# TheShadow29/VidSitu

Hardware: AMD Instinct MI355X
Metric: clips/s (10s@32x224x224) SlowFast+TxEnc fwd+bwd (higher is better)
Workload: dtype bf16

## Files before the change

include/vidsitu_hip.h:

```cpp
#ifndef VIDSITU_HIP_H
#define VIDSITU_HIP_H

#include <stddef.h>
#include <stdint.h>

#ifdef __cplusplus
extern "C" {
#endif

typedef enum vs_status {
  VS_OK = 0,
  VS_ERR_BAD_ARG = -1,
  VS_ERR_UNSUPPORTED = -2,
  VS_ERR_WORKSPACE = -3,
  VS_ERR_LAUNCH = -4
} vs_status;

#define VS_CONV_AFFINE 1
#define VS_CONV_RESIDUAL 2
#define VS_CONV_RELU 4
#define VS_CONV_STATS 8
#define VS_CONV_NAIVE 16
#define VS_CONV_TILE(id) (((id) + 1) << 8)
#define VS_CONV_RING(ns) (((ns) & 7) << 16)
// ... 78 lines not shown
  const float* gamma;
  const float* beta;
  float* stats_partial;
  const void* bn_y2;
  int bn_y2_ld;
  const float* mean2;
  const float* invstd2;
  float* stats_partial2;
} vs_dgrad_epilogue;
int vs_conv_dgrad_ex(const void* dy, const void* wt, void* dx, const vs_conv_desc* d,
                     const vs_dgrad_epilogue* ep, void* workspace, size_t ws_bytes, void* stream);
int vs_weight_transpose(const void* w, void* wt, int Cout, int taps, int Cin, void* stream);
int vs_weight_transpose_batched(const void* src, void* dst, const int64_t* table, int n,
                                int64_t total, void* stream);
int vs_transpose_f32_batched(const float* src, float* dst, const int64_t* table, int n, int64_t total,
                             void* stream);
int vs_weight_transpose_tiled(const void* src, void* dst, const int64_t* table, const int64_t* tile_first,
                              int n, int64_t total_tiles, int elem_bytes, void* stream);

#define VS_WGRAD_NODEEP (1 << 12)
#define VS_WGRAD_FORCEDEEP (1 << 13)
size_t vs_conv_wgrad_workspace_bytes(const vs_conv_desc* d);
int vs_conv_wgrad(const void* dy, const void* x, float* dw, const vs_conv_desc* d,
                  void* workspace, size_t ws_bytes, void* stream);
typedef struct vs_wgrad_item {
  const void* dy;
  const void* x;
  float* dw;
  vs_conv_desc d;
} vs_wgrad_item;
int vs_conv_wgrad_group_ok(const vs_wgrad_item* items, int n);
size_t vs_conv_wgrad_group_workspace_bytes(const vs_wgrad_item* items, int n);
int vs_conv_wgrad_group(const vs_wgrad_item* items, int n, void* workspace, size_t ws_bytes, void* stream);
int vs_conv_wgrad_partial(const void* dy, const void* x, float* dw, const vs_conv_desc* d, void* slabs,
                          size_t slab_bytes, int* splits, void* stream);
int64_t vs_wgrad_reduce_blocks(int64_t elements);
int vs_wgrad_reduce(const float* slabs, float* dw, int64_t elements, int splits, void* stream);
int vs_wgrad_reduce_batched(const int64_t* table, int n_entries, int64_t total_blocks, void* stream);
int vs_wgrad_reduce_defer(int mode);
int vs_wgrad_reduce_flush(void);

int vs_bn_finalize(const float* partials, int nparts, double count, const float* gamma,
                   const float* beta, float* running_mean, float* running_var, float momentum,
                   float eps, float* scale, float* shift, float* mean, float* invstd, int C,
                   void* stream);
size_t vs_bn_finalize_workspace_bytes(void);
int vs_bn_finalize_ws(const float* partials, int nparts, double count, const float* gamma, const float* beta,
                      float* running_mean, float* running_var, float momentum, float eps, float* scale,
                      float* shift, float* mean, float* invstd, int C, void* workspace, size_t ws_bytes,
                      void* stream);
int vs_bn_partials_reduce(const float* partials, int nparts, float* out, int C, int G,
                          void* stream);
int vs_bn_apply(const void* y, const float* scale, const float* shift, const void* residual,
                void* out, int64_t rows, int C, int y_ld, int res_ld, int out_ld, int relu,
                void* stream);
int vs_bn_apply_mask(const void* y, const float* scale, const float* shift, const void* residual,
                     void* out, uint8_t* relu_bits, int64_t rows, int C, int y_ld, int res_ld,
                     int out_ld, void* stream);
int vs_bn_apply2(const void* y, const float* scale, const float* shift, const void* y2, const float* scale2,
                 const float* shift2, void* out, uint8_t* relu_bits, int64_t rows, int C, int y_ld, int y2_ld,
                 int out_ld, void* stream);
int vs_bn_bwd_reduce(const void* dz, const void* z, const void* y, const float* mean,
                     const float* invstd, const float* gamma, const float* beta, float* partial,
                     int64_t rows, int C, int dz_ld, int z_ld, int y_ld, int relu, void* stream);
int vs_bn_bwd_reduce_rows(int64_t rows, int C);
int vs_bn_bwd_finalize(const float* partial, int nparts, float* dgamma, float* dbeta, int C,
// ... 170 lines not shown
```

vidsitu_amd/_lib.py:

```python
import ctypes as C
import os
import subprocess

_HERE = os.path.dirname(os.path.abspath(__file__))
LIB_PATH = os.environ.get("VS_LIB_PATH") or os.path.join(_HERE, "libvidsitu_hip.so")
CSRC_DIR = os.path.join(_HERE, "csrc")

VS_CONV_AFFINE = 1
VS_CONV_RESIDUAL = 2
VS_CONV_RELU = 4
VS_CONV_STATS = 8
VS_CONV_NAIVE = 16


class ConvDesc(C.Structure):

    _fields_ = [
        (n, C.c_int32)
        for n in (
            "N Ti Hi Wi Cin To Ho Wo Cout kT kH kW sT sH sW pT pH pW x_ld y_ld res_ld flags"
        ).split()
    ]


# ... 17 lines not shown
SIGNATURES = {
    "vs_last_error_string": (C.c_char_p, []),
    "vs_version": (_i, []),
    "vs_launch_count": (_i64, []),
    "vs_pack_input": (_i, [_p, _i, _p, _i, _i, _i, _i, _i, _i, _p]),
    "vs_frames_u8_pack": (_i, [_p, _p, _p, _i, _i, _i, _i, _i, _i, _p, _p, _i, _p]),
    "vs_stem_conv_fwd": (_i, [_p, _p, _p, _i, _i, _i, _i, _i, _i, _i, _i, _p, _p, _p, _p]),
    "vs_stem_stats_rows": (_i, [_i, _i, _i, _i]),
    "vs_stem_wgrad_workspace_bytes": (_sz, [_i, _i, _i, _i, _i, _i]),
    "vs_stem_conv_wgrad": (_i, [_p, _p, _p, _i, _i, _i, _i, _i, _i, _i, _p, _sz, _p]),
    "vs_conv_fwd": (_i, [_p, _p, _p, _dp, _p, _p, _p, _p, _p, _sz, _p]),
    "vs_conv_stats_rows": (_i, [_dp]),
    "vs_conv_workspace_bytes": (_sz, [_dp, _i]),
    "vs_conv_plan": (_i, [_dp, _i, _p]),
    "vs_conv_aol_ok": (_i, [_dp]),
    "vs_conv_fwd_aol": (_i, [_p, _p, _p, _dp, _p, _p, _p, _p]),
    "vs_conv_wgrad_aol_ok": (_i, [_dp]),
    "vs_conv_wgrad_aol": (_i, [_p, _p, _p, _dp, _p, _p, _p, _sz, _p]),
    "vs_conv_fwd_bc_fusable": (_i, [_dp, _i]),
    "vs_conv_fwd_bc": (_i, [_p, _p, _dp, _p, _p, _p, _i, _p, _p, _p, _i, _p, _i, _i, _p]),
    "vs_conv_dgrad": (_i, [_p, _p, _p, _dp, _p, _p, _sz, _p]),
    "vs_conv_dgrad_bnstats_rows": (_i, [_dp]),
    "vs_conv_dgrad_bnstats": (_i, [_p, _p, _p, _dp, _p, _p, _i, _p, _p, _p, _p, _p, _p, _p, _sz, _p]),
    "vs_conv_dgrad_ex": (_i, [_p, _p, _p, _dp, C.POINTER(DgradEpilogue), _p, _sz, _p]),
    "vs_weight_transpose": (_i, [_p, _p, _i, _i, _i, _p]),
    "vs_weight_transpose_batched": (_i, [_p, _p, _p, _i, _i64, _p]),
    "vs_transpose_f32_batched": (_i, [_p, _p, _p, _i, _i64, _p]),
    "vs_weight_transpose_tiled": (_i, [_p, _p, _p, _p, _i, _i64, _i, _p]),
    "vs_conv_wgrad_workspace_bytes": (_sz, [_dp]),
    "vs_conv_wgrad": (_i, [_p, _p, _p, _dp, _p, _sz, _p]),
    "vs_conv_wgrad_group_ok": (_i, [C.POINTER(WgradItem), _i]),
    "vs_conv_wgrad_group_workspace_bytes": (_sz, [C.POINTER(WgradItem), _i]),
    "vs_conv_wgrad_group": (_i, [C.POINTER(WgradItem), _i, _p, _sz, _p]),
    "vs_conv_wgrad_partial": (_i, [_p, _p, _p, _dp, _p, _sz, C.POINTER(C.c_int), _p]),
    "vs_wgrad_reduce_blocks": (_i64, [_i64]),
    "vs_wgrad_reduce": (_i, [_p, _p, _i64, _i, _p]),
    "vs_wgrad_reduce_batched": (_i, [_p, _i, _i64, _p]),
    "vs_wgrad_reduce_defer": (_i, [_i]),
    "vs_wgrad_reduce_flush": (_i, []),
    "vs_bn_finalize": (_i, [_p, _i, _d, _p, _p, _p, _p, _f, _f, _p, _p, _p, _p, _i, _p]),
    "vs_bn_finalize_workspace_bytes": (_sz, []),
    "vs_bn_finalize_ws": (_i, [_p, _i, _d, _p, _p, _p, _p, _f, _f, _p, _p, _p, _p, _i, _p, _sz, _p]),
    "vs_bn_bwd_finalize_ws": (_i, [_p, _i, _p, _p, _i, _p, _sz, _p]),
    "vs_bn_partials_reduce": (_i, [_p, _i, _p, _i, _i, _p]),
    "vs_bn_apply": (_i, [_p, _p, _p, _p, _p, _i64, _i, _i, _i, _i, _i, _p]),
    "vs_bn_apply_mask": (_i, [_p, _p, _p, _p, _p, _p, _i64, _i, _i, _i, _i, _p]),
    "vs_bn_apply2": (_i, [_p, _p, _p, _p, _p, _p, _p, _p, _i64, _i, _i, _i, _i, _p]),
    "vs_bn_bwd_reduce": (_i, [_p, _p, _p, _p, _p, _p, _p, _p, _i64, _i, _i, _i, _i, _i, _p]),
    "vs_bn_bwd_reduce_rows": (_i, [_i64, _i]),
    "vs_bn_bwd_finalize": (_i, [_p, _i, _p, _p, _i, _p]),
    "vs_bn_bwd_apply": (
        _i,
        [_p, _p, _p, _p, _p, _p, _p, _p, _p, _p, _p, _i64, _i, _i, _i, _i, _i, _i, _i, _p],
    ),
    "vs_bn_bwd_apply2": (_i, [_p] * 16 + [_i64, _i, _i, _i, _i, _i, _i, _p]),
    "vs_residual_add_f32": (_i, [_p, _p, _p, _p, _p, _i64, _i, _i, _i, _i, _i, _i, _p]),
    "vs_maxpool_hw3s2_fwd": (_i, [_p, _p, _p, _i, _i, _i, _i, _i, _i, _i, _p]),
    "vs_maxpool_hw3s2_bwd": (_i, [_p, _p, _p, _i, _i, _i, _i, _i, _i, _i, _p]),
    "vs_bn_apply_maxpool": (_i, [_p, _p, _p, _p, _p, _i, _i, _i, _i, _i, _i, _i, _p]),
    "vs_bn_bwd_reduce_pool": (_i, [_p, _p, _p, _p, _p, _p, _p, _p, _i, _i, _i, _i, _i, _i, _i, _p]),
    "vs_bn_bwd_apply_pool": (_i, [_p, _p, _p, _p, _p, _p, _p, _p, _p, _p, _i, _i, _i, _i, _i, _i, _i, _i, _p]),
    "vs_maxpool_t_fwd": (_i, [_p, _p, _p, _i, _i, _i, _i, _i, _p]),
    "vs_maxpool_t_bwd": (_i, [_p, _p, _p, _i, _i, _i, _i, _i, _p]),
    "vs_avgpool_fwd": (_i, [_p, _p, _i, _i64, _i, _i, _i, _i, _p]),
    "vs_avgpool_bwd": (_i, [_p, _p, _i, _i64, _i, _i, _i, _i, _p]),
    "vs_linear_fwd": (_i, [_p, _p, _p, _p, _i, _i, _i, _i, _p]),
# ... 111 lines not shown
```

vidsitu_amd/csrc/conv_wgrad.hip:

```cpp
#include <stdlib.h>

#include "common.h"

#include <mutex>
#include <type_traits>
#include "glue_bodies.h"

typedef __attribute__((ext_vector_type(4))) short s16x4;
typedef __attribute__((address_space(3))) s16x4 lds_s16x4;

struct WgradP {
  const uint16_t* dy;
  const uint16_t* x;
  float* out;
  int P;
  int Cout, Kp, Cin, x_ld, dy_ld;
  int To, Ho, Wo, Ti, Hi, Wi;
  int kT, kH, kW, sT, sH, sW, pT, pH, pW;
  int tilesM, tilesN, S, rows_per_split;
  unsigned x_bytes, dy_bytes;
  int xcd_order;
  int dbg;
  const float* in_scale;
  const float* in_shift;
};

#define WG_OOB 0x80000000u

#define WG_ROWTAB 1024

__device__ __forceinline__ int wg_swz_chunk(int row) {
  return ((row & 3) << 1) | (((row >> 3) & 1) << 3);
}

template <int BM, int BN, int WM, int WN, int MODE>
__global__ __launch_bounds__(256) void conv_wgrad_kernel(WgradP p) {
  extern __shared__ __attribute__((aligned(16))) char smem[];
  constexpr int TM = BM / WM, TN = BN / WN;
  constexpr int MR = TM / 16, NR = TN / 16;
  constexpr int CM = BM / 8, CN = BN / 8;
  constexpr int RPM = 256 / CM, RPN = 256 / CN;
  constexpr int IM = (64 + RPM - 1) / RPM, IN = (64 + RPN - 1) / RPN;
  constexpr int IMG = 64 * 256;
  constexpr int STAGE = 2 * IMG;
  static_assert(WM * WN == 4, "4 waves");

  const int tid = threadIdx.x;
  int bid = blockIdx.x;
  if (p.xcd_order) {
    const int nwg = gridDim.x, q = nwg >> 3, r = nwg & 7, xcd = blockIdx.x & 7;
    bid = (xcd < r ? xcd * (q + 1) : r * (q + 1) + (xcd - r) * q) + (blockIdx.x >> 3);
  }
  const int ntile = p.tilesM * p.tilesN;
  const int s = bid / ntile;
  bid -= s * ntile;
  const int tn = bid % p.tilesN, tm = bid / p.tilesN;
  const int m0 = tm * BM, n0 = tn * BN;
  const int pbeg = s * p.rows_per_split;
  const int pend = min(p.P, pbeg + p.rows_per_split);

  int4* rowtab = (int4*)(smem + 2 * STAGE);

  const int ccm = tid % CM, rm = tid / CM;
  const int ccn = tid % CN, rn = tid / CN;
  const bool mcol_ok = (m0 + ccm * 8) < p.Cout;
  const int ncol = n0 + ccn * 8;
  const bool ncol_ok = ncol < p.Kp;
  int dt = 0, dh = 0, dw = 0, c0 = 0;
  if (MODE == 1 && ncol_ok) {
    const int tap = ncol / p.Cin;
    c0 = ncol - tap * p.Cin;
    dw = tap % p.kW;
    const int t2 = tap / p.kW;
    dh = t2 % p.kH;
    dt = t2 / p.kH;
  }

  u32x4 ra[IM], rb[IN];
  const __amdgpu_buffer_rsrc_t xsrc =
      __builtin_amdgcn_make_buffer_rsrc((void*)p.x, 0, (int)p.x_bytes, 0x00020000);
  const __amdgpu_buffer_rsrc_t dysrc =
      __builtin_amdgcn_make_buffer_rsrc((void*)p.dy, 0, (int)p.dy_bytes, 0x00020000);
  const unsigned dycol = (unsigned)((m0 + ccm * 8) * 2);
  const unsigned xtap = (MODE == 1)
// ... 117 lines not shown
      }
      __syncthreads();
    }
    const int nsteps = (cend - chunk0 + 63) >> 6;
    gload(chunk0, chunk0);
    __syncthreads();
    sstore(0);
    __syncthreads();
    for (int st = 0; st < nsteps - 1; ++st) {
      const int cur = st & 1;
      gload(chunk0 + (st + 1) * 64, chunk0);
      __builtin_amdgcn_sched_barrier(0);
      compute(cur);
      __builtin_amdgcn_sched_barrier(0);
      sstore(cur ^ 1);
      __syncthreads();
    }
    compute((nsteps - 1) & 1);
    __syncthreads();
  }

  float* dst = p.out + (long long)s * p.Cout * p.Kp;
#pragma unroll
  for (int a = 0; a < MR; ++a)
#pragma unroll
    for (int b = 0; b < NR; ++b) {
      const int col = n0 + wn * TN + b * 16 + li;
#pragma unroll
      for (int r = 0; r < 4; ++r) {
        const int row = m0 + wm * TM + a * 16 + g * 4 + r;
        if (row < p.Cout && col < p.Kp) dst[(long long)row * p.Kp + col] = acc[a][b][r];
      }
    }
}

template <int BM, int BN, int WM, int WN, int MODE, int NS, bool AOL = false, int ROWS = 64>
__device__ __forceinline__ void conv_wgrad_ring_body(const WgradP& p, const int blk, const int nblk) {
  static_assert(!AOL || MODE == 0, "apply on load: pointwise launches");
  static_assert(ROWS == 64, "stage depth (the half-depth variant of round 4 was measured slower and removed)");
  extern __shared__ __attribute__((aligned(16))) char smem[];
  constexpr int TM = BM / WM, TN = BN / WN;
  constexpr int MR = TM / 16, NR = TN / 16;
  constexpr int CM = BM / 8, CN = BN / 8;
  constexpr int IMG = ROWS * 256;
  constexpr int STAGE = 2 * IMG;
  constexpr int D = NS - 1;
  constexpr int RG = ROWS / 16;
  constexpr int L = 2 * RG;
  constexpr int SPC = WG_ROWTAB / ROWS;
  static_assert(WM * WN == 4, "4 waves");
  static_assert((D - 1) * L <= 63, "vmcnt range");

  const int tid = threadIdx.x;
  int bid = blk;
  if (p.xcd_order) {
    const int nwg = nblk, q = nwg >> 3, r = nwg & 7, xcd = blk & 7;
    bid = (xcd < r ? xcd * (q + 1) : r * (q + 1) + (xcd - r) * q) + (blk >> 3);
  }
  const int ntile = p.tilesM * p.tilesN;
  const int s = bid / ntile;
  bid -= s * ntile;
  const int tn = bid % p.tilesN, tm = bid / p.tilesN;
  const int m0 = tm * BM, n0 = tn * BN;
  const int pbeg = s * p.rows_per_split;
  const int pend = min(p.P, pbeg + p.rows_per_split);
  const int nsteps = (pend - pbeg + ROWS - 1) / ROWS;
// ... 1051 lines not shown
      int mx = 0;
      for (int x = 0; x < 8; ++x) {
        long long sl = 0;
        for (long long c = x; c < chunks; c += 8) sl = (c >> 3) * 32 + ((c == chunks - 1 && (pos & 31)) ? (pos & 31) : 32);
        g.jobend[x] = (unsigned short)sl;
        if ((int)sl > mx) mx = (int)sl;
      }
#ifdef VS_WGG_DEBUG
      for (int x = 0; x < 8; ++x) {
        fprintf(stderr, "xcd %d (%d slots):", x, (int)g.jobend[x]);
        for (int i = 0; i < cnt[x]; ++i) fprintf(stderr, " [slot %u p %u s %u t %u]", g.jobtab[x][i] >> 23, (g.jobtab[x][i] >> 18) & 31, (g.jobtab[x][i] >> 12) & 63, g.jobtab[x][i] & 4095);
        fprintf(stderr, "\n");
      }
      for (int a = 0; a < n; ++a) fprintf(stderr, "problem %d: tiles %d x %d S %d rps %d count %d\n", a, g.p[a].tilesM, g.p[a].tilesN, g.p[a].S, g.p[a].rows_per_split, g.count[a]);
#endif
      g.jobs = 1;
      grid = 8 * mx;
    }
  }
  static std::once_flag gattr;
  std::call_once(gattr, [] {
    (void)hipFuncSetAttribute((const void*)conv_wgrad_deep_group_kernel, hipFuncAttributeMaxDynamicSharedMemorySize, 160 * 1024);
  });
  const size_t smem = (size_t)WGD_NU * WGD_UNIT + 2 * WGD_TAB * sizeof(int2);
  hipLaunchKernelGGL(conv_wgrad_deep_group_kernel, dim3(grid), dim3(512), smem, (hipStream_t)stream, g);
  VS_CHECK_LAUNCH();
  if (r.n > 0) {
    hipLaunchKernelGGL(wgrad_reduce_group_kernel, dim3((unsigned)r.first[r.n]), dim3(256), 0, (hipStream_t)stream, r);
    VS_CHECK_LAUNCH();
  }
  return VS_OK;
}

static int wgrad_impl(const void* dy, const void* x, float* dw, const vs_conv_desc* d, void* workspace,
                      size_t ws_bytes, void* stream, bool reduce_now, int* splits_out,
                      const float* in_scale = nullptr, const float* in_shift = nullptr) {
  VS_CHECK_ARG(d && dy && x && dw, "null argument");
  VS_CHECK_ARG(d->Cin % 8 == 0 && d->Cout % 8 == 0, "Cin and Cout must be multiples of 8");
  VS_CHECK_ARG(d->x_ld % 8 == 0 && d->y_ld % 8 == 0, "row pitches must be multiples of 8");
  VS_CHECK_ARG((long long)d->N * d->Ti * d->Hi * d->Wi < (1ll << 31), "too many positions");
  const WgCfg c = wg_pick(d);
  const size_t need = vs_conv_wgrad_workspace_bytes(d);
  if (need > 0 && (workspace == nullptr || ws_bytes < need)) {
    vs_set_error("vs_conv_wgrad: workspace too small (%zu < %zu)", ws_bytes, need);
    return VS_ERR_WORKSPACE;
  }
  if (g_pending.have && ((const void*)g_pending.r.slabs == workspace || g_pending.r.dw == dw)) pending_flush();
  if (in_scale && !wgrad_aol_plan_ok(d)) {
    vs_set_error("vs_conv_wgrad_aol: apply on load is not built for this weight gradient (ask vs_conv_wgrad_aol_ok)");
    return VS_ERR_UNSUPPORTED;
  }
  WgradP p;
  {
    const int rc = wg_fill_params(p, dy, x, c.S > 1 ? (float*)workspace : dw, d, c);
    if (rc) return rc;
  }
  p.in_scale = in_scale;
  p.in_shift = in_shift;
  {
    static const int xo = [] { const char* e = getenv("VS_WGRAD_XCD"); return e ? atoi(e) : 1; }();
    p.xcd_order = xo && (c.tilesM * c.tilesN <= 32 || xo == 2 || (c.S % 8 == 0 && c.tilesM * c.tilesN <= 64));
    static const int dbg = [] { const char* e = getenv("VS_WGRAD_DBG"); return e ? atoi(e) : 0; }();
    p.dbg = dbg;
  }
  p.rows_per_split = c.rows_per_split;
  const bool dense = (d->kT * d->kH * d->kW == 1) && d->sT == 1 && d->sH == 1 && d->sW == 1 &&
                     d->pT == 0 && d->pH == 0 && d->pW == 0;
  const int mode = dense ? 0 : 1;
  hipStream_t st = (hipStream_t)stream;
  const int fring = (d->flags >> 16) & 7;
  int ring = fring == 1 ? 0 : (fring >= 2 ? (fring > 3 ? 3 : fring) : (c.bm == 128 ? 2 : 0));
  if (d->kT * d->kH * d->kW > 31) ring = 0;
  int rc;
  if (c.deep) {
    static std::once_flag dattr;
    std::call_once(dattr, [] {
      (void)hipFuncSetAttribute((const void*)conv_wgrad_deep_kernel<0, false>, hipFuncAttributeMaxDynamicSharedMemorySize, 160 * 1024);
      (void)hipFuncSetAttribute((const void*)conv_wgrad_deep_kernel<1, false>, hipFuncAttributeMaxDynamicSharedMemorySize, 160 * 1024);
      (void)hipFuncSetAttribute((const void*)conv_wgrad_deep_kernel<0, true>, hipFuncAttributeMaxDynamicSharedMemorySize, 160 * 1024);
      (void)hipFuncSetAttribute((const void*)conv_wgrad_deep_kernel<1, true>, hipFuncAttributeMaxDynamicSharedMemorySize, 160 * 1024);
    });
    static const int stag = [] { const char* e = getenv("VS_WGRAD_DEEP_STAG"); return e ? atoi(e) : 1; }();
    if (in_scale) {
      vs_set_error("vs_conv_wgrad_aol: not built for the deep-pipeline plan");
      return VS_ERR_UNSUPPORTED;
    }
    const size_t smem = (size_t)WGD_NU * WGD_UNIT + 2 * WGD_TAB * sizeof(int2);
    const int grid = p.tilesM * p.tilesN * p.S;
    if (stag && mode == 0) hipLaunchKernelGGL((conv_wgrad_deep_kernel<0, true>), dim3(grid), dim3(512), smem, st, p);
    else if (stag) hipLaunchKernelGGL((conv_wgrad_deep_kernel<1, true>), dim3(grid), dim3(512), smem, st, p);
    else if (mode == 0) hipLaunchKernelGGL((conv_wgrad_deep_kernel<0, false>), dim3(grid), dim3(512), smem, st, p);
    else hipLaunchKernelGGL((conv_wgrad_deep_kernel<1, false>), dim3(grid), dim3(512), smem, st, p);
    VS_CHECK_LAUNCH();
    rc = VS_OK;
// ... 43 lines not shown
```

vidsitu_amd/ops.py:

```python
import ctypes as C

import torch

from . import _lib
from ._lib import (
    VS_CONV_AFFINE,
    VS_CONV_NAIVE,
    VS_CONV_RELU,
    VS_CONV_RESIDUAL,
    VS_CONV_STATS,
    ConvDesc,
)

BF16 = torch.bfloat16


def _stream():
    return C.c_void_p(torch.cuda.current_stream().cuda_stream)


def _ptr(t):
    if t is None:
        return None
    if not t.is_cuda:
# ... 479 lines not shown
    return lambda: _lib.call("vs_wgrad_reduce", _ptr(ws), _ptr(out), n, S, _stream())


WGRAD_GROUP_MAX = 20


def _wgrad_items(items):
    arr = (_lib.WgradItem * len(items))()
    for i, (dy, x, k, s, p, out) in enumerate(items):
        if not out.permute(0, 2, 3, 4, 1).is_contiguous() or out.dtype != torch.float32:
            raise _lib.VsError("conv_wgrad out must be fp32 with [Cout][taps][Cin] memory")
        arr[i].dy, arr[i].x, arr[i].dw = dy.data_ptr(), x.data_ptr(), out.data_ptr()
        arr[i].d = make_desc(x.shape, act_ld(x), dy.shape, act_ld(dy), k, s, p, 0)
        _ptr(dy), _ptr(x), _ptr(out)
    return arr


def conv_wgrad_group_ok(items):
    if not 1 <= len(items) <= WGRAD_GROUP_MAX:
        return False
    return bool(_lib.load().vs_conv_wgrad_group_ok(_wgrad_items(items), len(items)))


def conv_wgrad_group(items):
    if _WHATIF_WGRAD:
        return
    arr = _wgrad_items(items)
    need = int(_lib.load().vs_conv_wgrad_group_workspace_bytes(arr, len(items)))
    ws = _workspace(need, items[0][0].device, "wgrad") if need else None
    _lib.call("vs_conv_wgrad_group", arr, len(items), _ptr(ws), C.c_size_t(ws.numel() if ws is not None else 0),
              _stream())


def conv_wgrad(dy, x, k, s, p, out=None, ring=0, batch=None, tile=None, slots=0, deep=True):
    cout, cin = dy.shape[1], x.shape[1]
    if out is None:
        out = torch.empty((cout, *k, cin), dtype=torch.float32, device=x.device).permute(0, 4, 1, 2, 3)
    elif not out.permute(0, 2, 3, 4, 1).is_contiguous() or out.dtype != torch.float32:
        raise _lib.VsError("conv_wgrad out must be fp32 with [Cout][taps][Cin] memory")
    if batch is not None:
        return batch.wgrad(dy, x, k, s, p, out, ring)
    if _WHATIF_WGRAD:
        return out
    flags = ((ring & 7) << 16) | (((tile + 1) << 8) if tile is not None else 0) | (((slots // 8) & 0xff) << 24)
    if not deep:
        flags |= 1 << 12
    elif deep == "force":
        flags |= 1 << 13
    d = make_desc(x.shape, act_ld(x), dy.shape, act_ld(dy), k, s, p, flags)
    need = _lib.load().vs_conv_wgrad_workspace_bytes(C.byref(d))
    ws = _workspace(need, x.device, "wgrad") if need else None
    _lib.call("vs_conv_wgrad", _ptr(dy), _ptr(x), _ptr(out), C.byref(d), _ptr(ws),
              C.c_size_t(ws.numel() if ws is not None else 0), _stream())
    return out


import os as _os
_WHATIF = int(_os.environ.get("VS_WHATIF", "0"))
_BN_TWO_LEVEL = int(_os.environ.get("VS_BN_TWO_LEVEL", "512"))
BN_FIN2 = _os.environ.get("VS_BN_FIN2", "1") != "0"
_fin_ws = [0]
_whatif_const = {}


def _fin_ws_bytes():
    if not _fin_ws[0]:
# ... 781 lines not shown
```

vidsitu_amd/trunk.py:

```python
import contextlib
import os

import torch
from torch import nn

from . import ops

STAGE_DEPTH = {50: (3, 4, 6, 3), 101: (3, 4, 23, 3), "tiny": (1, 0, 0, 1), "mini": (1, 1, 1, 1)}
TEMPORAL_KERNEL_BASIS = {
    "c2d": [[[1]], [[1]], [[1]], [[1]], [[1]]],
    "i3d": [[[5]], [[3]], [[3, 1]], [[3, 1]], [[1, 3]]],
    "slow": [[[1]], [[1]], [[1]], [[3]], [[3]]],
    "slowfast": [[[1], [5]], [[1], [3]], [[1], [3]], [[3], [3]], [[3], [3]]],
}
POOL1 = {
    "c2d": [[2, 1, 1]],
    "i3d": [[2, 1, 1]],
    "slow": [[1, 1, 1]],
    "slowfast": [[1, 1, 1], [1, 1, 1]],
}


class Conv3dP(nn.Module):

# ... 471 lines not shown
            else:
                sc = _Unit.fwd(self.branch1, self.branch1_bn, x, False, train=train, saved=saved)
        a = _Unit.fwd(b2.a, b2.a_bn, x, True, train=train, saved=saved)
        if sc_aff is not None:
            b = _Unit.fwd(b2.b, b2.b_bn, a, True, train=True, saved=saved)
            z = _Unit.fwd(b2.c, b2.c_bn, b, True, out=out, train=True, saved=saved, residual_affine=sc_aff)
            if saved is not None and len(saved) >= 4:
                saved[-1]["sc_rec"] = saved[-4]
            return z
        if train and self._aol_ok(a, saved):
            yb, aff = _Unit.fwd(b2.b, b2.b_bn, a, True, train=True, saved=saved, no_apply=True)
            z = _Unit.fwd(b2.c, b2.c_bn, yb, True, residual=sc, out=out, train=True, saved=saved, x_affine=aff)
            if self.has_sc and saved is not None and len(saved) >= 4:
                saved[-1]["sc_rec"] = saved[-4]
            return z
        if not train and self._bc_fusable(a):
            (sb, hb), (s_c, h_c) = b2.b_bn.fold, b2.c_bn.fold
            return ops.conv_fwd_bc(a, b2.b.w_bf16, b2.b.k, b2.b.s, b2.b.p, sb, hb, b2.c.w_bf16, s_c, h_c,
                                   residual=sc, relu=True, out=out)
        b = _Unit.fwd(b2.b, b2.b_bn, a, True, train=train, saved=saved)
        if ResBlock.residual_fp32 and not train:
            branch = _Unit.fwd(b2.c, b2.c_bn, b, False, train=False)
            res = sc if self.has_sc else getattr(x, "_vs_f32", x)
            z, z32 = ops.residual_add_f32(branch, res, relu=True, out16=out)
            z._vs_f32 = z32
            return z
        z = _Unit.fwd(b2.c, b2.c_bn, b, True, residual=sc, out=out, train=train, saved=saved)
        if self.has_sc and train and saved is not None and len(saved) >= 4:
            saved[-1]["sc_rec"] = saved[-4]
        return z

    def bwd(self, saved, dout, chain=False, carry=None):
        rc, rb, ra = saved.pop(), saved.pop(), saved.pop()
        sink = [] if self._wgrad_grouped(rc, rb, ra, saved[-1] if (self.has_sc and saved) else None, dout) else None
        res = self._bwd_units(saved, dout, chain, rc, rb, ra, sink)
        if sink:
            items = [(dy, x, c.k, c.s, c.p, c.weight.grad) for dy, x, c in sink]
            if carry is None:
                ops.conv_wgrad_group(items)
            else:
                carry["items"] += items
                carry["blocks"] += 1
                if carry["blocks"] >= ResBlock.group_span or len(carry["items"]) + 4 > ops.WGRAD_GROUP_MAX:
                    ResBlock.flush_wgrads(carry)
        return res

    @staticmethod
    def flush_wgrads(carry):
        if carry and carry["items"]:
            items = carry["items"]
            ops.conv_wgrad_group(items)
        if carry:
            carry["items"], carry["blocks"] = [], 0


    group_span = int(os.environ.get("VS_WGRAD_GROUP_SPAN", "3"))

    group_wgrads = os.environ.get("VS_WGRAD_GROUP", "1") != "0"
    group_max_positions = int(os.environ.get("VS_WGRAD_GROUP_MAXP", "1000000000"))
    group_min_channels = int(os.environ.get("VS_WGRAD_GROUP_MINC", "128"))

    def _wgrad_grouped(self, rc, rb, ra, rsc, dout):
        if (not ResBlock.group_wgrads or not dout.is_cuda or _Unit.wgrad_batch is not None or _Unit.split_wgrad_reduce
                or ResBlock.aol):
            return False
        recs = [r for r in (rc, rb, ra, rsc) if r is not None]
        key = ("wgg",) + tuple(tuple(r["y"].shape) for r in recs)
        hit = self.__dict__.setdefault("_bc_ok", {}).get(key)
        if hit is None:
            hit = True
            items = []
            for r in recs:
                c, y, x = r["conv"], r["y"], r["x"]
                if (c.is_stem or c.cin_pad != c.cin or c.bias is not None or r.get("x_affine") is not None
                        or c.cout < ResBlock.group_min_channels or not isinstance(x, torch.Tensor)
                        or not getattr(c.weight, "_vs_direct_grad", True)):
                    hit = False
                    break
                items.append((y, x, c.k, c.s, c.p, torch.empty(0)))
            if hit:
                hit = min(ops.act_rows(r["y"]) for r in recs) <= ResBlock.group_max_positions
            if hit:
                probe = [(y, x, k, s_, p, torch.empty((y.shape[1], *k, x.shape[1]), dtype=torch.float32,
                                                      device=y.device).permute(0, 4, 1, 2, 3)) for y, x, k, s_, p, _ in items]
                hit = ops.conv_wgrad_group_ok(probe)
            self._bc_ok[key] = hit
        return hit

    def _bwd_units(self, saved, dout, chain, rc, rb, ra, sink):
        cbits = rc.get("zbits")
        dy_sc = None
        if (self.has_sc and cbits is not None and ResBlock.fuse_sc_bwd and dout.is_cuda and saved
                and rc["conv"].bias is None and saved[-1]["conv"].bias is None and ops.bn_apply2_ok(rc["y"].shape[1])):
            rsc = saved[-1]
            units = []
            for r in (rc, rsc):
                bn = r["bn"]
                if bn.weight.grad is None:
                    bn.weight.grad = torch.zeros_like(bn.weight)
                if bn.bias.grad is None:
                    bn.bias.grad = torch.zeros_like(bn.bias)
                ops.bn_bwd_sums(dout, r["y"], r["mean"], r["invstd"], cbits, bn.weight.grad, bn.bias.grad,
                                partial=r.pop("bwd_partial", None))
                units.append((r["y"], r["mean"], r["invstd"], bn.weight, bn.weight.grad, bn.bias.grad))
            dy_c, dy_sc = ops.bn_bwd_apply2(dout, cbits, units[0], units[1])
            db, g = _Unit.bwd(rc, dout, producer=rb, dy_ready=dy_c, wgrad_sink=sink)
        else:
            db, g = _Unit.bwd(rc, dout, want_dres=cbits is None, producer=rb, wgrad_sink=sink)
        da, _ = _Unit.bwd(rb, db, producer=ra, wgrad_sink=sink)
        if self.has_sc:
            rsc = saved.pop()
            if ResBlock.accumulate_shortcut:
                dxa, _ = _Unit.bwd(ra, da, wgrad_sink=sink)
                if cbits is not None:
                    dx, _ = _Unit.bwd(rsc, dout, dz_bits=cbits, dx_residual=dxa, inplace=True, dy_ready=dy_sc, wgrad_sink=sink)
                else:
                    dx, _ = _Unit.bwd(rsc, g, masked=True, dx_residual=dxa, inplace=True, wgrad_sink=sink)
            else:
# ... 605 lines not shown
            par = self._fork_ctx(d[0].device)
            d_in = list(d)
            par.fork()
            for p in reversed(range(self.num_pathways)):
                with par.on(p):
                    if p == 1 and late is not None:
                        d[1] = late()
                    getattr(self.s1, f"pathway{p}_stem").bwd(saved, d[p])
            par.join(keep=d_in)
            assert not saved, "trunk backward did not consume every saved record"

    def _backward_stage(self, st, k):
        saved, d = st["saved"], st["d"]
        P = self.num_pathways
        stage = getattr(self, f"s{k}")
        fuse = getattr(self, f"s{k}_fuse", None) if self.multi else None
        if k == 2:
            for p in reversed(range(P)):
                if self.pool1[p][0] > 1:
                    rec = saved.pop()
                    d[p] = ops.maxpool_t_bwd(d[p], rec["tpool_idx"], rec["tpool_in"], rec["kt"])
        late = None
        if fuse is not None:
            d, late = self._fuse_bwd(saved, d, defer=VideoTrunk.fuse_on_fast)
        par = self._fork_ctx(d[0].device)
        d_in = list(d)
        par.fork()
        for p in reversed(range(P)):
            with par.on(p):
                if p == 1 and late is not None:
                    d[1] = late()
                g = d[p]
                blks = stage.blocks(p)
                carry = {"items": [], "blocks": 0}
                for i in reversed(range(len(blks))):
                    if isinstance(blks[i], ResBlock):
                        g = blks[i].bwd(saved, g, chain=i > 0, carry=carry)
                    else:
                        ResBlock.flush_wgrads(carry)
                        g = blks[i].bwd(saved, g)
                ResBlock.flush_wgrads(carry)
                d[p] = g
        par.join(keep=d_in)
        st["d"] = d

    fuse_on_fast = os.environ.get("VS_FUSE_ON_FAST", "1") != "0"

    def _fuse_bwd(self, saved, d, defer=False):
        d_cat, d_fast = d
        rec = saved.pop()
        cf = rec["conv"].cout
        cs = d_cat.shape[1] - cf
        run = lambda: _Unit.bwd(rec, ops.channel_slice(d_cat, cs, cf), dx_residual=d_fast)[0]
        if defer:
            return [ops.channel_slice(d_cat, 0, cs), None], run
        return [ops.channel_slice(d_cat, 0, cs), run()], None
```

Before: 730.2.

## Group narrow-channel wgrad convs into one multi-body kernel launch

Adds a grouped weight-gradient kernel that dispatches each block to one of several templated tile bodies, so ResBlocks whose channel count is below the wide-group threshold can batch their wgrad convolutions. Items are sorted by work size and launched together, followed by a single grouped split-K reduce, or one reduce per item. The Python side classifies blocks as wide or narrow, carries narrow items across blocks and flushes whenever the kind changes. The goal is fewer kernel launches and better GPU fill for the small fast-pathway convs, at the cost of a kernel with many bodies and possibly higher register and LDS use.

```diff
diff --git a/include/vidsitu_hip.h b/include/vidsitu_hip.h
--- a/include/vidsitu_hip.h
+++ b/include/vidsitu_hip.h
@@ -134,6 +134,11 @@
 int vs_conv_wgrad_group_ok(const vs_wgrad_item* items, int n);
 size_t vs_conv_wgrad_group_workspace_bytes(const vs_wgrad_item* items, int n);
 int vs_conv_wgrad_group(const vs_wgrad_item* items, int n, void* workspace, size_t ws_bytes, void* stream);
+#define VS_WGS_REDUCE_EACH 1
+int vs_conv_wgrad_group_small_ok(const vs_wgrad_item* items, int n);
+size_t vs_conv_wgrad_group_small_workspace_bytes(const vs_wgrad_item* items, int n);
+int vs_conv_wgrad_group_small(const vs_wgrad_item* items, int n, void* workspace, size_t ws_bytes, int flags,
+                              void* stream);
 int vs_conv_wgrad_partial(const void* dy, const void* x, float* dw, const vs_conv_desc* d, void* slabs,
                           size_t slab_bytes, int* splits, void* stream);
 int64_t vs_wgrad_reduce_blocks(int64_t elements);
diff --git a/vidsitu_amd/_lib.py b/vidsitu_amd/_lib.py
--- a/vidsitu_amd/_lib.py
+++ b/vidsitu_amd/_lib.py
@@ -73,6 +73,9 @@
     "vs_conv_wgrad_group_ok": (_i, [C.POINTER(WgradItem), _i]),
     "vs_conv_wgrad_group_workspace_bytes": (_sz, [C.POINTER(WgradItem), _i]),
     "vs_conv_wgrad_group": (_i, [C.POINTER(WgradItem), _i, _p, _sz, _p]),
+    "vs_conv_wgrad_group_small_ok": (_i, [C.POINTER(WgradItem), _i]),
+    "vs_conv_wgrad_group_small_workspace_bytes": (_sz, [C.POINTER(WgradItem), _i]),
+    "vs_conv_wgrad_group_small": (_i, [C.POINTER(WgradItem), _i, _p, _sz, _i, _p]),
     "vs_conv_wgrad_partial": (_i, [_p, _p, _p, _dp, _p, _sz, C.POINTER(C.c_int), _p]),
     "vs_wgrad_reduce_blocks": (_i64, [_i64]),
     "vs_wgrad_reduce": (_i, [_p, _p, _i64, _i, _p]),
diff --git a/vidsitu_amd/csrc/conv_wgrad.hip b/vidsitu_amd/csrc/conv_wgrad.hip
--- a/vidsitu_amd/csrc/conv_wgrad.hip
+++ b/vidsitu_amd/csrc/conv_wgrad.hip
@@ -34,7 +34,7 @@
 }
 
 template <int BM, int BN, int WM, int WN, int MODE>
-__global__ __launch_bounds__(256) void conv_wgrad_kernel(WgradP p) {
+__device__ __forceinline__ void conv_wgrad_body(const WgradP& p, const int blk, const int nblk) {
   extern __shared__ __attribute__((aligned(16))) char smem[];
   constexpr int TM = BM / WM, TN = BN / WN;
   constexpr int MR = TM / 16, NR = TN / 16;
@@ -46,10 +46,10 @@
   static_assert(WM * WN == 4, "4 waves");
 
   const int tid = threadIdx.x;
-  int bid = blockIdx.x;
+  int bid = blk;
   if (p.xcd_order) {
-    const int nwg = gridDim.x, q = nwg >> 3, r = nwg & 7, xcd = blockIdx.x & 7;
-    bid = (xcd < r ? xcd * (q + 1) : r * (q + 1) + (xcd - r) * q) + (blockIdx.x >> 3);
+    const int nwg = nblk, q = nwg >> 3, r = nwg & 7, xcd = blk & 7;
+    bid = (xcd < r ? xcd * (q + 1) : r * (q + 1) + (xcd - r) * q) + (blk >> 3);
   }
   const int ntile = p.tilesM * p.tilesN;
   const int s = bid / ntile;
@@ -233,6 +233,11 @@
         if (row < p.Cout && col < p.Kp) dst[(long long)row * p.Kp + col] = acc[a][b][r];
       }
     }
+}
+
+template <int BM, int BN, int WM, int WN, int MODE>
+__global__ __launch_bounds__(256) void conv_wgrad_kernel(WgradP p) {
+  conv_wgrad_body<BM, BN, WM, WN, MODE>(p, blockIdx.x, gridDim.x);
 }
 
 template <int BM, int BN, int WM, int WN, int MODE, int NS, bool AOL = false, int ROWS = 64>
@@ -1350,6 +1355,177 @@
   return VS_OK;
 }
 
+static int wg_xcd_order(const WgCfg& c) {
+  static const int xo = [] { const char* e = getenv("VS_WGRAD_XCD"); return e ? atoi(e) : 1; }();
+  return xo && (c.tilesM * c.tilesN <= 32 || xo == 2 || (c.S % 8 == 0 && c.tilesM * c.tilesN <= 64));
+}
+
+#define WGS_MAX 20
+struct WgSmallGroupP {
+  int n;
+  int first[WGS_MAX + 1];
+  int count[WGS_MAX];
+  int body[WGS_MAX];
+  WgradP p[WGS_MAX];
+};
+static_assert(sizeof(WgSmallGroupP) <= 4096, "kernel arguments");
+static_assert(WGS_MAX <= WGG_MAX, "one wgrad_reduce_group_kernel launch holds the slabs of a whole group");
+
+__global__ __launch_bounds__(256) void conv_wgrad_small_group_kernel(WgSmallGroupP g) {
+  const int b = blockIdx.x;
+  int j = 0;
+#pragma unroll
+  for (int i = 1; i < WGS_MAX; ++i)
+    if (i < g.n && b >= g.first[i]) j = i;
+  j = __builtin_amdgcn_readfirstlane(j);
+  const int blk = b - g.first[j], cnt = g.count[j];
+  if (blk >= cnt) return;
+  switch (__builtin_amdgcn_readfirstlane(g.body[j])) {
+    case 0: conv_wgrad_body<16, 64, 1, 4, 1>(g.p[j], blk, cnt); break;
+    case 1: conv_wgrad_body<16, 128, 1, 4, 1>(g.p[j], blk, cnt); break;
+    case 2: conv_wgrad_body<32, 64, 1, 4, 0>(g.p[j], blk, cnt); break;
+    case 3: conv_wgrad_body<32, 64, 1, 4, 1>(g.p[j], blk, cnt); break;
+    case 4: conv_wgrad_body<64, 64, 2, 2, 0>(g.p[j], blk, cnt); break;
+    case 5: conv_wgrad_body<64, 64, 2, 2, 1>(g.p[j], blk, cnt); break;
+    case 6: conv_wgrad_body<64, 128, 2, 2, 0>(g.p[j], blk, cnt); break;
+    case 7: conv_wgrad_body<64, 128, 2, 2, 1>(g.p[j], blk, cnt); break;
+    case 8: conv_wgrad_ring_body<128, 64, 2, 2, 0, 2>(g.p[j], blk, cnt); break;
+    case 9: conv_wgrad_ring_body<128, 64, 2, 2, 1, 2>(g.p[j], blk, cnt); break;
+    case 10: conv_wgrad_ring_body<128, 128, 2, 2, 1, 2>(g.p[j], blk, cnt); break;
+    default: break;
+  }
+}
+
+static int wgs_body(const WgCfg& c, int mode) {
+  static const int tab[][4] = {{16, 64, 1, 0},  {16, 128, 1, 1}, {32, 64, 0, 2},  {32, 64, 1, 3},
+                               {64, 64, 0, 4},  {64, 64, 1, 5},  {64, 128, 0, 6}, {64, 128, 1, 7},
+                               {128, 64, 0, 8}, {128, 64, 1, 9}, {128, 128, 1, 10}};
+  if (c.deep) return -1;
+  for (const auto& t : tab)
+    if (t[0] == c.bm && t[1] == c.bn && t[2] == mode) return t[3];
+  return -1;
+}
+
+static bool wg_dense(const vs_conv_desc* d) {
+  return (d->kT * d->kH * d->kW == 1) && d->sT == 1 && d->sH == 1 && d->sW == 1 && d->pT == 0 && d->pH == 0 &&
+         d->pW == 0;
+}
+
+static bool wgs_plan(const vs_wgrad_item* it, int n, WgCfg* cfg, int* body, size_t* slab_off, size_t* slab_total,
+                     int* order, size_t* smem) {
+  if (it == nullptr || n < 1 || n > WGS_MAX) return false;
+  size_t off = 0, lds = 0;
+  long long key[WGS_MAX], blocks = 0;
+  for (int j = 0; j < n; ++j) {
+    const vs_conv_desc* d = &it[j].d;
+    if (d->flags != 0 || d->Cin % 8 != 0 || d->Cout % 8 != 0 || d->x_ld % 8 != 0 || d->y_ld % 8 != 0) return false;
+    if ((long long)d->N * d->Ti * d->Hi * d->Wi >= (1ll << 31)) return false;
+    const int taps = d->kT * d->kH * d->kW;
+    const long long P = (long long)d->N * d->To * d->Ho * d->Wo;
+    const long long xb = (long long)d->N * d->Ti * d->Hi * d->Wi * d->x_ld * 2, db = P * d->y_ld * 2;
+    if (taps > 31 || P < 1 || xb >= (1ll << 31) || db >= (1ll << 31)) return false;
+    cfg[j] = wg_pick(d);
+    const int mode = wg_dense(d) ? 0 : 1;
+    body[j] = wgs_body(cfg[j], mode);
+    if (body[j] < 0) return false;
+    slab_off[j] = off;
+    if (cfg[j].S > 1) off += (size_t)cfg[j].S * d->Cout * taps * d->Cin * sizeof(float);
+    const size_t need = 2 * 2 * 64 * 256 + (mode ? 2 * WG_ROWTAB * sizeof(int2) : 0);
+    if (need > lds) lds = need;
+    const long long nb = (long long)cfg[j].tilesM * cfg[j].tilesN * cfg[j].S;
+    blocks += (nb + 7) / 8 * 8;
+    key[j] = (long long)cfg[j].rows_per_split * (cfg[j].bm + cfg[j].bn);
+    order[j] = j;
+  }
+  for (int a = 0; a < n; ++a)
+    for (int b = a + 1; b < n; ++b)
+      if (key[order[b]] > key[order[a]]) { const int t = order[a]; order[a] = order[b]; order[b] = t; }
+  *slab_total = off;
+  *smem = lds;
+  return blocks < (1ll << 31);
+}
+
+extern "C" int vs_conv_wgrad_group_small_ok(const vs_wgrad_item* items, int n) {
+  WgCfg cfg[WGS_MAX];
+  int body[WGS_MAX], order[WGS_MAX];
+  size_t off[WGS_MAX], tot, smem;
+  return wgs_plan(items, n, cfg, body, off, &tot, order, &smem) ? 1 : 0;
+}
+
+extern "C" size_t vs_conv_wgrad_group_small_workspace_bytes(const vs_wgrad_item* items, int n) {
+  WgCfg cfg[WGS_MAX];
+  int body[WGS_MAX], order[WGS_MAX];
+  size_t off[WGS_MAX], tot = 0, smem;
+  if (!wgs_plan(items, n, cfg, body, off, &tot, order, &smem)) return 0;
+  return tot;
+}
+
+extern "C" int vs_conv_wgrad_group_small(const vs_wgrad_item* items, int n, void* workspace, size_t ws_bytes, int flags,
+                                         void* stream) {
+  VS_CHECK_ARG(items != nullptr && n >= 1 && n <= WGS_MAX, "1 .. 20 items");
+  VS_CHECK_ARG((flags & ~VS_WGS_REDUCE_EACH) == 0, "unknown flags");
+  WgCfg cfg[WGS_MAX];
+  int body[WGS_MAX], order[WGS_MAX];
+  size_t off[WGS_MAX], tot = 0, smem = 0;
+  if (!wgs_plan(items, n, cfg, body, off, &tot, order, &smem)) {
+    vs_set_error("vs_conv_wgrad_group_small: an item's plan is not one of the grouped bodies (ask vs_conv_wgrad_group_small_ok)");
+    return VS_ERR_UNSUPPORTED;
+  }
+  if (tot > 0 && (workspace == nullptr || ws_bytes < tot)) {
+    vs_set_error("vs_conv_wgrad_group_small: workspace too small (%zu < %zu)", ws_bytes, tot);
+    return VS_ERR_WORKSPACE;
+  }
+  if (g_pending.have) pending_flush();
+  WgSmallGroupP g;
+  WgReduceGroupP r;
+  g.n = n;
+  r.n = 0;
+  r.first[0] = 0;
+  int first = 0;
+  for (int a = 0; a < n; ++a) {
+    const int j = order[a];
+    const vs_wgrad_item& t = items[j];
+    VS_CHECK_ARG(t.dy && t.x && t.dw, "null tensor");
+    const vs_conv_desc* d = &t.d;
+    float* out = cfg[j].S > 1 ? (float*)((char*)workspace + off[j]) : t.dw;
+    const int rc = wg_fill_params(g.p[a], t.dy, t.x, out, d, cfg[j]);
+    if (rc) return rc;
+    g.p[a].xcd_order = wg_xcd_order(cfg[j]);
+    g.body[a] = body[j];
+    g.first[a] = first;
+    g.count[a] = cfg[j].tilesM * cfg[j].tilesN * cfg[j].S;
+    first += (g.count[a] + 7) / 8 * 8;
+    if (cfg[j].S > 1) {
+      const int e = r.n++;
+      r.slabs[e] = out;
+      r.dw[e] = t.dw;
+      r.len[e] = (long long)d->Cout * g.p[a].Kp;
+      r.S[e] = cfg[j].S;
+      r.first[e + 1] = r.first[e] + wgrad_reduce_vblocks(r.len[e], r.S[e]);
+    }
+  }
+  for (int j = n; j <= WGS_MAX; ++j) g.first[j] = first;
+  for (int j = n; j < WGS_MAX; ++j) g.count[j] = 0, g.body[j] = -1;
+  static std::once_flag sattr;
+  std::call_once(sattr, [] {
+    (void)hipFuncSetAttribute((const void*)conv_wgrad_small_group_kernel, hipFuncAttributeMaxDynamicSharedMemorySize,
+                              160 * 1024);
+  });
+  hipLaunchKernelGGL(conv_wgrad_small_group_kernel, dim3(first), dim3(256), smem, (hipStream_t)stream, g);
+  VS_CHECK_LAUNCH();
+  if (r.n > 0 && (flags & VS_WGS_REDUCE_EACH)) {
+    for (int e = 0; e < r.n; ++e) {
+      hipLaunchKernelGGL(wgrad_reduce_kernel, dim3((unsigned)wgrad_reduce_vblocks(r.len[e], r.S[e])), dim3(256), 0,
+                         (hipStream_t)stream, r.slabs[e], r.dw[e], r.len[e], r.S[e]);
+      VS_CHECK_LAUNCH();
+    }
+  } else if (r.n > 0) {
+    hipLaunchKernelGGL(wgrad_reduce_group_kernel, dim3((unsigned)r.first[r.n]), dim3(256), 0, (hipStream_t)stream, r);
+    VS_CHECK_LAUNCH();
+  }
+  return VS_OK;
+}
+
 static int wgrad_impl(const void* dy, const void* x, float* dw, const vs_conv_desc* d, void* workspace,
                       size_t ws_bytes, void* stream, bool reduce_now, int* splits_out,
                       const float* in_scale = nullptr, const float* in_shift = nullptr) {
@@ -1376,8 +1552,7 @@
   p.in_scale = in_scale;
   p.in_shift = in_shift;
   {
-    static const int xo = [] { const char* e = getenv("VS_WGRAD_XCD"); return e ? atoi(e) : 1; }();
-    p.xcd_order = xo && (c.tilesM * c.tilesN <= 32 || xo == 2 || (c.S % 8 == 0 && c.tilesM * c.tilesN <= 64));
+    p.xcd_order = wg_xcd_order(c);
     static const int dbg = [] { const char* e = getenv("VS_WGRAD_DBG"); return e ? atoi(e) : 0; }();
     p.dbg = dbg;
   }
diff --git a/vidsitu_amd/ops.py b/vidsitu_amd/ops.py
--- a/vidsitu_amd/ops.py
+++ b/vidsitu_amd/ops.py
@@ -535,6 +535,22 @@
               _stream())
 
 
+def conv_wgrad_group_small_ok(items):
+    if not 1 <= len(items) <= WGRAD_GROUP_MAX:
+        return False
+    return bool(_lib.load().vs_conv_wgrad_group_small_ok(_wgrad_items(items), len(items)))
+
+
+def conv_wgrad_group_small(items):
+    if _WHATIF_WGRAD:
+        return
+    arr = _wgrad_items(items)
+    need = int(_lib.load().vs_conv_wgrad_group_small_workspace_bytes(arr, len(items)))
+    ws = _workspace(need, items[0][0].device, "wgrad") if need else None
+    _lib.call("vs_conv_wgrad_group_small", arr, len(items), _ptr(ws), C.c_size_t(ws.numel() if ws is not None else 0),
+              0 if REDUCE_MERGE else 1, _stream())
+
+
 def conv_wgrad(dy, x, k, s, p, out=None, ring=0, batch=None, tile=None, slots=0, deep=True):
     cout, cin = dy.shape[1], x.shape[1]
     if out is None:
diff --git a/vidsitu_amd/trunk.py b/vidsitu_amd/trunk.py
--- a/vidsitu_amd/trunk.py
+++ b/vidsitu_amd/trunk.py
@@ -527,24 +527,42 @@
 
     def bwd(self, saved, dout, chain=False, carry=None):
         rc, rb, ra = saved.pop(), saved.pop(), saved.pop()
-        sink = [] if self._wgrad_grouped(rc, rb, ra, saved[-1] if (self.has_sc and saved) else None, dout) else None
+        kind = self._wgrad_grouped(rc, rb, ra, saved[-1] if (self.has_sc and saved) else None, dout)
+        if kind == "narrow" and carry is not None and not carry.get("narrow", True):
+            kind = False
+        sink = [] if kind else None
         res = self._bwd_units(saved, dout, chain, rc, rb, ra, sink)
         if sink:
             items = [(dy, x, c.k, c.s, c.p, c.weight.grad) for dy, x, c in sink]
             if carry is None:
-                ops.conv_wgrad_group(items)
+                ResBlock._launch_group(kind, items)
             else:
-                carry["items"] += items
-                carry["blocks"] += 1
-                if carry["blocks"] >= ResBlock.group_span or len(carry["items"]) + 4 > ops.WGRAD_GROUP_MAX:
-                    ResBlock.flush_wgrads(carry)
+                ResBlock._carry_add(carry, kind, items)
         return res
+
+    @staticmethod
+    def _carry_add(carry, kind, items):
+        if carry["items"] and (carry.get("kind", "wide") != kind
+                               or len(carry["items"]) + len(items) > ops.WGRAD_GROUP_MAX):
+            ResBlock.flush_wgrads(carry)
+        carry["items"] += items
+        carry["blocks"] += 1
+        carry["kind"] = kind
+        if kind == "wide" and (carry["blocks"] >= ResBlock.group_span or len(carry["items"]) + 4 > ops.WGRAD_GROUP_MAX):
+            ResBlock.flush_wgrads(carry)
+
+    @staticmethod
+    def _launch_group(kind, items):
+        if kind == "narrow":
+            ops.conv_wgrad_group_small(items)
+        else:
+            ops.conv_wgrad_group(items)
 
     @staticmethod
     def flush_wgrads(carry):
         if carry and carry["items"]:
             items = carry["items"]
-            ops.conv_wgrad_group(items)
+            ResBlock._launch_group(carry.get("kind", "wide"), items)
         if carry:
             carry["items"], carry["blocks"] = [], 0
 
@@ -554,31 +572,37 @@
     group_wgrads = os.environ.get("VS_WGRAD_GROUP", "1") != "0"
     group_max_positions = int(os.environ.get("VS_WGRAD_GROUP_MAXP", "1000000000"))
     group_min_channels = int(os.environ.get("VS_WGRAD_GROUP_MINC", "128"))
+    group_narrow = os.environ.get("VS_WGRAD_GROUP_NARROW", "1") != "0"
+    group_narrow_slow = os.environ.get("VS_WGRAD_GROUP_NARROW_SLOW", "1") != "0"
 
     def _wgrad_grouped(self, rc, rb, ra, rsc, dout):
         if (not ResBlock.group_wgrads or not dout.is_cuda or _Unit.wgrad_batch is not None or _Unit.split_wgrad_reduce
                 or ResBlock.aol):
             return False
         recs = [r for r in (rc, rb, ra, rsc) if r is not None]
-        key = ("wgg",) + tuple(tuple(r["y"].shape) for r in recs)
+        key = ("wgg", ResBlock.group_narrow) + tuple(tuple(r["y"].shape) for r in recs)
         hit = self.__dict__.setdefault("_bc_ok", {}).get(key)
         if hit is None:
-            hit = True
+            hit = "wide"
             items = []
             for r in recs:
                 c, y, x = r["conv"], r["y"], r["x"]
                 if (c.is_stem or c.cin_pad != c.cin or c.bias is not None or r.get("x_affine") is not None
-                        or c.cout < ResBlock.group_min_channels or not isinstance(x, torch.Tensor)
-                        or not getattr(c.weight, "_vs_direct_grad", True)):
+                        or not isinstance(x, torch.Tensor) or not getattr(c.weight, "_vs_direct_grad", True)):
                     hit = False
                     break
+                if c.cout < ResBlock.group_min_channels:
+                    hit = "narrow"
                 items.append((y, x, c.k, c.s, c.p, torch.empty(0)))
-            if hit:
-                hit = min(ops.act_rows(r["y"]) for r in recs) <= ResBlock.group_max_positions
+            if hit == "narrow" and not ResBlock.group_narrow:
+                hit = False
+            if hit == "wide":
+                hit = "wide" if min(ops.act_rows(r["y"]) for r in recs) <= ResBlock.group_max_positions else False
             if hit:
                 probe = [(y, x, k, s_, p, torch.empty((y.shape[1], *k, x.shape[1]), dtype=torch.float32,
                                                       device=y.device).permute(0, 4, 1, 2, 3)) for y, x, k, s_, p, _ in items]
-                hit = ops.conv_wgrad_group_ok(probe)
+                ok = ops.conv_wgrad_group_small_ok if hit == "narrow" else ops.conv_wgrad_group_ok
+                hit = hit if ok(probe) else False
             self._bc_ok[key] = hit
         return hit
 
@@ -1250,7 +1274,7 @@
                     d[1] = late()
                 g = d[p]
                 blks = stage.blocks(p)
-                carry = {"items": [], "blocks": 0}
+                carry = {"items": [], "blocks": 0, "narrow": ResBlock.group_narrow_slow or (P > 1 and p == 1)}
                 for i in reversed(range(len(blks))):
                     if isinstance(blks[i], ResBlock):
                         g = blks[i].bwd(saved, g, chain=i > 0, carry=carry)
```

New measurement: 736.5, median of 6. No clear change (+0.9%).
